# HudsonAlpha/rust-msbwt

Hardware: AMD Instinct MI355X
Metric: k-mer count queries/sec (whole node) (higher is better)
Workload: dtype u64

## Files before the change

### include/msbwt_hip.h

```cpp
#ifndef MSBWT_HIP_H
#define MSBWT_HIP_H

#include <stddef.h>
#include <stdint.h>

#ifdef __cplusplus
extern "C" {
#endif

#define MSBWT_VC_LEN 6
#define MSBWT_LETTER_BITS 3
#define MSBWT_NUMBER_BITS 5
#define MSBWT_NUM_POWER 32
#define MSBWT_MASK 0x07
#define MSBWT_COUNT_MASK 0x1F

#define MSBWT_OK 0
#define MSBWT_ERR_IO (-1)
#define MSBWT_ERR_UNEXPECTED_EOF (-2)
#define MSBWT_ERR_BAD_HEADER (-3)
#define MSBWT_ERR_INVALID_SYMBOL (-4)
#define MSBWT_ERR_INVALID_RANGE (-5)
#define MSBWT_ERR_HIP (-6)
#define MSBWT_ERR_NOT_LOADED (-7)
// ... 184 lines not shown
int msbwt_sparse_filter_bits(uint64_t tag, uint32_t *word, uint32_t *mask);
int msbwt_rle_set_query_length(msbwt_rle *bwt, int k);
int msbwt_rle_get_query_length(const msbwt_rle *bwt);
int msbwt_auto_sparse_max_depth(int query_length);
size_t msbwt_rle_download_sparse_table(const msbwt_rle *bwt, void *out_lines, size_t cap_bytes, void *out_side, size_t cap_side_bytes);
int msbwt_rle_set_presence_filter(msbwt_rle *bwt, int mode);
int msbwt_rle_get_presence_filter(const msbwt_rle *bwt);
int msbwt_rle_set_pair_index(msbwt_rle *bwt, int mode);
int msbwt_rle_get_pair_index(const msbwt_rle *bwt);
int msbwt_rle_set_pair_stride(msbwt_rle *bwt, int stride);
int msbwt_rle_get_pair_stride(const msbwt_rle *bwt);
double msbwt_rle_get_typical_range_width(const msbwt_rle *bwt);
int msbwt_auto_pair_stride(uint64_t total_symbols, uint64_t free_hbm_bytes, uint64_t hbm_total_bytes, double typical_width, int *stride);
int msbwt_rle_set_memory_budget(msbwt_rle *bwt, uint64_t bytes);
uint64_t msbwt_rle_get_memory_budget(const msbwt_rle *bwt);
int msbwt_auto_index_plan(uint64_t total_symbols, uint64_t free_hbm_bytes, uint64_t hbm_total_bytes, double typical_width, uint64_t budget_bytes,
                          int *pair_index, int *pair_stride, int *flat_depth, int *packed_depth, uint64_t *index_bytes);
int msbwt_run_build_fits_device(uint64_t total_symbols, uint64_t free_hbm_bytes);
int msbwt_rle_set_block_format(msbwt_rle *bwt, int format);
int msbwt_rle_get_block_format(const msbwt_rle *bwt);
int msbwt_rle_set_search_kernel(msbwt_rle *bwt, int mode);
int msbwt_rle_get_search_kernel(const msbwt_rle *bwt);
int msbwt_rle_search_kernel_for(const msbwt_rle *bwt, size_t k);
#define MSBWT_SEARCH_COUNTERS 16
int msbwt_rle_set_search_counters(msbwt_rle *bwt, int enabled);
int msbwt_rle_search_counters(const msbwt_rle *bwt, uint64_t *out, void *hip_stream);
int msbwt_rle_set_line_streaming(msbwt_rle *bwt, int mode);
int msbwt_rle_get_line_streaming(const msbwt_rle *bwt);
int msbwt_rle_probe_line_rate(const msbwt_rle *bwt, int which, double *lines_per_second);
uint64_t msbwt_rle_device_bytes(const msbwt_rle *bwt);
int msbwt_rle_kernel_time_ms(const msbwt_rle *bwt, double *avg_ms, uint64_t *launches);
int msbwt_rle_set_kernel_timing(msbwt_rle *bwt, int enabled);
int msbwt_rle_device_ordinal(const msbwt_rle *bwt);
const char *msbwt_rle_last_error(const msbwt_rle *bwt);
size_t msbwt_build_plane_blocks(const uint8_t *rle_bytes, size_t len, void *out_blocks, size_t cap_blocks,
                                uint64_t *out_total);
size_t msbwt_build_run_blocks(const uint8_t *rle_bytes, size_t len, void *out_blocks, size_t cap_blocks,
                              void *out_overflow, size_t cap_overflow, uint64_t *out_total, uint64_t *out_noverflow);
size_t msbwt_rle_download_blocks(const msbwt_rle *bwt, void *out_blocks, size_t cap_blocks);
const char *msbwt_version(void);

size_t msbwt_convert_to_vec(const uint8_t *ascii, size_t n, uint8_t *out, size_t cap);
int msbwt_save_bwt_numpy(const uint8_t *rle_bytes, size_t n, const char *utf8_path);
int msbwt_save_bwt_runs_numpy(const uint8_t *syms, const uint64_t *counts, size_t nruns,
                              const char *utf8_path);
void msbwt_convert_stoi(const uint8_t *ascii, size_t n, uint8_t *out_codes);
// ... 8 lines not shown
```

### include/msbwt_hip.hpp

```cpp
#pragma once

#include <algorithm>
#include <array>
#include <cstdint>
#include <stdexcept>
#include <string>
#include <system_error>
#include <vector>

#include "msbwt_hip.h"

namespace msbwt {

constexpr std::size_t VC_LEN = MSBWT_VC_LEN;
constexpr std::size_t LETTER_BITS = MSBWT_LETTER_BITS;
constexpr std::size_t NUMBER_BITS = MSBWT_NUMBER_BITS;
constexpr std::size_t NUM_POWER = MSBWT_NUM_POWER;
constexpr std::uint8_t MASK = MSBWT_MASK;
constexpr std::uint8_t COUNT_MASK = MSBWT_COUNT_MASK;

struct BWTRange {
    std::uint64_t l = 0;
    std::uint64_t h = 0;
    bool operator==(const BWTRange &o) const { return l == o.l && h == o.h; }
// ... 427 lines not shown
    }
    void device_status(void *hip_stream = nullptr) const { check(msbwt_rle_device_status(raw_, hip_stream)); }
    void allgather_counts(void *comm, const void *d_mine, std::size_t n_mine, void *d_all, int wire_bits = 64,
                          void *hip_stream = nullptr) const {
        check(msbwt_rle_allgather_counts(raw_, comm, d_mine, n_mine, d_all, wire_bits, hip_stream));
    }

    void set_table_depth(int depth) { check(msbwt_rle_set_table_depth(raw_, depth)); }
    void set_table_packed(int mode) { check(msbwt_rle_set_table_packed(raw_, mode)); }
    void set_pair_index(int mode) { check(msbwt_rle_set_pair_index(raw_, mode)); }
    void set_search_kernel(int mode) { check(msbwt_rle_set_search_kernel(raw_, mode)); }
    void set_memory_budget(std::uint64_t bytes) { check(msbwt_rle_set_memory_budget(raw_, bytes)); }
    void set_batch_order(int mode) { check(msbwt_rle_set_batch_order(raw_, mode)); }
    void set_sparse_table(int depth) { check(msbwt_rle_set_sparse_table(raw_, depth)); }
    void set_query_length(int k) { check(msbwt_rle_set_query_length(raw_, k)); }
    int get_query_length() const { return msbwt_rle_get_query_length(raw_); }
    void set_sparse_tiers(int mode) { check(msbwt_rle_set_sparse_tiers(raw_, mode)); }
    bool get_sparse_tiers() const { return msbwt_rle_get_sparse_tiers(raw_) != 0; }
    void set_sparse_second(int mode) { check(msbwt_rle_set_sparse_second(raw_, mode)); }
    int get_sparse_table() const { return msbwt_rle_get_sparse_table(raw_); }
    void set_table_side(int mode) { check(msbwt_rle_set_table_side(raw_, mode)); }
    std::uint64_t device_bytes() const { return msbwt_rle_device_bytes(raw_); }
    int search_kernel_for(size_t k) const { return msbwt_rle_search_kernel_for(raw_, k); }
    msbwt_rle *raw() const { return raw_; }

    RleBWT replicate(int device) const {
        msbwt_rle *other = msbwt_rle_replicate(raw_, device);
        if (!other) throw Panic(MSBWT_ERR_HIP, msbwt_rle_last_error(raw_));
        return RleBWT(other);
    }
    static std::vector<std::uint64_t> count_kmers_multi(const std::vector<const RleBWT *> &replicas,
                                                        const std::vector<std::uint8_t> &kmers, std::size_t k) {
        if (replicas.empty()) throw std::invalid_argument("no replicas");
        const std::size_t n = k ? kmers.size() / k : 0;
        std::vector<const msbwt_rle *> raws;
        for (const RleBWT *r : replicas) raws.push_back(r->raw_);
        std::vector<std::uint64_t> out(n);
        const int code = msbwt_rle_count_kmers_multi(raws.data(), raws.size(), kmers.data(), k, n, out.data());
        if (code != MSBWT_OK) throw Panic(code, "count_kmers_multi failed");
        return out;
    }

  private:
    explicit RleBWT(msbwt_rle *adopted) : raw_(adopted) {}
    void check(int code) const {
        if (code == MSBWT_OK) return;
// ... 61 lines not shown
```

### rust-msbwt_amd/_build.py

```python
import os
import subprocess
import sys

HERE = os.path.dirname(os.path.abspath(__file__))
CSRC = os.path.join(HERE, "csrc")
LIB = os.path.join(HERE, "libmsbwt_hip.so")
SOURCES = ["capi.cpp", "index_build.cpp", "query.cpp", "sources.cpp", "spectrum.cpp", "produce.cpp", "multi_device.cpp", "kernels.hip", "lanes.hip", "lanes_tier.hip", "lanes_wide.hip", "lanes_xwide.hip", "extend.hip", "sparse_table.hip", "device_build.hip", "pair_index.hip", "gather.hip", "order.hip", "run_build.hip", "reads_build.hip", "run_encode.hip", "merge.hip", "merge_many.hip", "source_index.hip", "spectrum.hip", "canonical.hip", "source_spectrum.hip", "kmer_graph.hip", "plane_index.cpp", "run_index.cpp", "npy_io.cpp", "rle_codec.cpp"]
HEADERS = ["handle.hpp", "index_build.hpp", "kernels.hpp", "lanes_kernel.hpp", "sparse_table.hpp", "sparse_build.hpp", "sparse_policy.hpp", "device_build.hpp", "pair_index.hpp", "gather.hpp", "order.hpp", "run_build.hpp", "reads_build.hpp", "run_encode.hpp", "workgroup.hpp", "rle_subruns.hpp", "merge.hpp", "merge_common.hpp", "source_index.hpp", "source_count.hpp", "source_spectrum.hpp", "kmer_graph.hpp", "frontier.hpp", "frontier_walk.hpp", "spectrum.hpp", "canonical.hpp", "rank_ops.hpp", "search_common.hpp", "host_pipeline.hpp", "plane_index.hpp", "run_index.hpp", "table_policy.hpp", "npy_io.hpp", "rle_codec.hpp", os.path.join("..", "..", "include", "msbwt_hip.h")]


def hipcc():
    for cand in (os.environ.get("HIPCC"), "/opt/rocm/bin/hipcc", "hipcc"):
        if cand and (os.path.isabs(cand) and os.path.exists(cand) or not os.path.isabs(cand)):
            return cand
    return "hipcc"


def stale():
    if not os.path.exists(LIB):
        return True
    t = os.path.getmtime(LIB)
    deps = [os.path.join(CSRC, f) for f in SOURCES + HEADERS] + [os.path.abspath(__file__)]
    return any(os.path.getmtime(d) > t for d in deps)


def build(force=False, verbose=False):
    if not force and not stale():
        return LIB
    from concurrent.futures import ThreadPoolExecutor

    objdir = os.path.join(HERE, "build")
# ... 31 lines not shown
```

### rust-msbwt_amd/_lib.py

```python
import ctypes as C
import os

HERE = os.path.dirname(os.path.abspath(__file__))
LIB_PATH = os.path.join(HERE, "libmsbwt_hip.so")

OK = 0
ERR_IO, ERR_UNEXPECTED_EOF, ERR_BAD_HEADER, ERR_INVALID_SYMBOL = -1, -2, -3, -4
ERR_INVALID_RANGE, ERR_HIP, ERR_NOT_LOADED, ERR_TOO_LARGE, ERR_INVALID_ARG, ERR_INTERNAL = -5, -6, -7, -8, -9, -10
ERR_OVERFLOW, ERR_RCCL = -11, -12
COMM_ID_BYTES = 128
SPARSE_INFO_WORDS = 120
BUILD_STAGES = ("copy_in", "read_order", "histogram", "collect", "sort", "emit", "encode", "copy_out")
MERGE_MAX_INPUTS = 32
SOURCE_INDEX_SLACK = 1024
SPECTRUM_INFO_WORDS = 40
SPECTRUM_MIN_FRONTIER = 64
MERGE_STAGES = ("copy_in", "decode", "iterate", "emit", "encode", "copy_out")

SIZE_MAX = C.c_size_t(-1).value

_vp, _u8, _u64, _sz, _int = C.c_void_p, C.c_uint8, C.c_uint64, C.c_size_t, C.c_int
_pu64 = C.POINTER(C.c_uint64)
SIGNATURES = {
    "msbwt_rle_new": (_vp, [_u8]),
# ... 87 lines not shown
    "msbwt_rle_get_memory_budget": (_u64, [_vp]),
    "msbwt_auto_index_plan": (_int, [_u64, _u64, _u64, C.c_double, _u64, C.POINTER(C.c_int), C.POINTER(C.c_int), C.POINTER(C.c_int), C.POINTER(C.c_int), _pu64]),
    "msbwt_rle_set_table_side": (_int, [_vp, _int]),
    "msbwt_rle_table_info": (_int, [_vp, _pu64, _pu64, _pu64]),
    "msbwt_rle_set_sparse_table": (_int, [_vp, _int]),
    "msbwt_rle_get_sparse_table": (_int, [_vp]),
    "msbwt_rle_sparse_table_info": (_int, [_vp, _pu64]),
    "msbwt_sparse_hash": (_int, [_u64, _int, _u64, C.POINTER(C.c_uint32), C.POINTER(C.c_uint32)]),
    "msbwt_sparse_table_shape": (_int, [_int, _u64, _pu64, C.POINTER(C.c_int)]),
    "msbwt_sparse_hash64": (_int, [_u64, _int, _u64, C.POINTER(C.c_uint32), _pu64]),
    "msbwt_auto_sparse_depth": (_int, [_pu64, _pu64, _int, _u64, _int, C.POINTER(C.c_int), _pu64]),
    "msbwt_rle_download_sparse_table": (_sz, [_vp, _vp, _sz, _vp, _sz]),
    "msbwt_allgather_piece_queries": (_sz, [_sz, _int]),
    "msbwt_rle_set_search_counters": (_int, [_vp, _int]),
    "msbwt_rle_search_counters": (_int, [_vp, _vp, _vp]),
    "msbwt_rle_set_presence_filter": (_int, [_vp, _int]),
    "msbwt_rle_get_presence_filter": (_int, [_vp]),
    "msbwt_run_build_fits_device": (_int, [_u64, _u64]),
    "msbwt_rle_set_block_format": (_int, [_vp, _int]),
    "msbwt_rle_get_block_format": (_int, [_vp]),
    "msbwt_rle_set_search_kernel": (_int, [_vp, _int]),
    "msbwt_rle_get_search_kernel": (_int, [_vp]),
    "msbwt_rle_search_kernel_for": (_int, [_vp, _sz]),
    "msbwt_rle_set_pair_index": (_int, [_vp, _int]),
    "msbwt_rle_get_pair_index": (_int, [_vp]),
    "msbwt_rle_set_pair_stride": (_int, [_vp, _int]),
    "msbwt_rle_get_pair_stride": (_int, [_vp]),
    "msbwt_rle_get_typical_range_width": (C.c_double, [_vp]),
    "msbwt_auto_pair_stride": (_int, [_u64, _u64, _u64, C.c_double, C.POINTER(C.c_int)]),
    "msbwt_rle_set_sparse_tiers": (_int, [_vp, _int]),
    "msbwt_rle_get_sparse_tiers": (_int, [_vp]),
    "msbwt_rle_set_sparse_second": (_int, [_vp, _int]),
    "msbwt_auto_sparse_choice": (_int, [_pu64, _pu64, _pu64, _int, _u64, _int, _int, C.POINTER(C.c_int), C.POINTER(C.c_int), _pu64]),
    "msbwt_sparse_filter_bits": (_int, [_u64, C.POINTER(C.c_uint32), C.POINTER(C.c_uint32)]),
    "msbwt_rle_set_query_length": (_int, [_vp, _int]),
    "msbwt_rle_get_query_length": (_int, [_vp]),
    "msbwt_auto_sparse_max_depth": (_int, [_int]),
    "msbwt_rle_set_line_streaming": (_int, [_vp, _int]),
    "msbwt_rle_get_line_streaming": (_int, [_vp]),
    "msbwt_rle_probe_line_rate": (_int, [_vp, _int, C.POINTER(C.c_double)]),
    "msbwt_rle_device_bytes": (_u64, [_vp]),
    "msbwt_rle_kernel_time_ms": (_int, [_vp, C.POINTER(C.c_double), _pu64]),
    "msbwt_rle_set_kernel_timing": (_int, [_vp, _int]),
    "msbwt_rle_device_ordinal": (_int, [_vp]),
    "msbwt_rle_last_error": (C.c_char_p, [_vp]),
    "msbwt_version": (C.c_char_p, []),
# ... 50 lines not shown
```

### rust-msbwt_amd/csrc/capi.cpp

```cpp
#include <algorithm>
#include <cstdint>
#include <cstdio>
#include <cstdlib>
#include <cstring>
#include <mutex>
#include <string>
#include <vector>

#include "handle.hpp"
#include "index_build.hpp"
#include "npy_io.hpp"
#include "pair_index.hpp"
#include "plane_index.hpp"
#include "run_index.hpp"
#include "sparse_table.hpp"

namespace {

constexpr int kMaxTableDepth = 16;
static_assert(MSBWT_SEARCH_COUNTERS == kSearchCounters, "the header's counter block is the kernels'");
static_assert(MSBWT_BUILD_STAGES == kReadsBuildStages, "the header's stage count is the builder's");
static_assert(MSBWT_MERGE_STAGES == kMergeStages, "the header's stage count is the merge's");
static_assert(MSBWT_MERGE_MAX_INPUTS == kMergeMaxInputs, "the header's input count is the merge's");
static_assert(10 + kSparseMaxDepth + 1 <= 42 && 45 + kSparseMaxDepth + 1 <= 80 && 80 + kSparseMaxDepth + 1 <= 112 && 119 <= MSBWT_SPARSE_INFO_WORDS,
              "msbwt_rle_sparse_table_info: [10 + d] distinct, [42] filtered, [45 + d] wide, [80 + d] once, [112] second tier, [113 .. 119) the walks");

const char *kVersion = "rust-msbwt_amd 0.1.0 (gfx950 plane-block index)";

double line_rate_of(const void *p, size_t bytes, hipStream_t stream) {
    hipEvent_t a = nullptr, b = nullptr;
    uint64_t lines = 0;
    float ms = 0.f;
    hipError_t e = hipEventCreate(&a);
    if (e == hipSuccess) e = hipEventCreate(&b);
    if (e == hipSuccess) e = launch_probe_lines(p, bytes, 4, nullptr, nullptr, stream);
    if (e == hipSuccess) e = hipEventRecord(a, stream);
    if (e == hipSuccess) e = launch_probe_lines(p, bytes, 48, &lines, nullptr, stream);
    if (e == hipSuccess) e = hipEventRecord(b, stream);
// ... 127 lines not shown
    if (device < 0 && hipGetDevice(&device) != hipSuccess) device = 0;
    h->device = device;
    if (const char *env = std::getenv("MSBWT_TABLE_DEPTH")) h->wanted_table_depth = std::max(-1, std::min(std::atoi(env), kMaxTableDepth));
    if (const char *env = std::getenv("MSBWT_TABLE_PACKED")) h->wanted_table_packed = std::atoi(env) ? 1 : 0;
    if (const char *env = std::getenv("MSBWT_TABLE_SIDE")) h->wanted_table_side = std::atoi(env) ? 1 : 0;
    if (const char *env = std::getenv("MSBWT_STREAM_LINES")) h->wanted_streaming = std::strcmp(env, "auto") == 0 ? -1 : (std::atoi(env) ? 1 : 0);
    if (const char *env = std::getenv("MSBWT_QUERY_K")) h->query_length = std::max(0, std::atoi(env));
    if (const char *env = std::getenv("MSBWT_SPARSE_TABLE")) {
        const int d = std::strcmp(env, "auto") == 0 ? -1 : std::atoi(env);
        h->wanted_sparse = (d == 0 || d == -1 || (d >= kSparseMinDepth && d <= kSparseMaxDepth)) ? d : -1;
    }
    if (const char *env = std::getenv("MSBWT_SPARSE_SECOND")) h->wanted_second = std::strcmp(env, "auto") == 0 ? -1 : (std::atoi(env) ? -1 : 0);
    if (const char *env = std::getenv("MSBWT_SPARSE_TIERS")) h->wanted_tiers = std::strcmp(env, "auto") == 0 ? -1 : (std::atoi(env) ? 1 : 0);
    if (const char *env = std::getenv("MSBWT_PAIR_INDEX")) h->wanted_pair = std::atoi(env) ? 1 : 0;
    if (const char *env = std::getenv("MSBWT_PAIR_STRIDE")) h->wanted_pair_stride = std::atoi(env);
    if (const char *env = std::getenv("MSBWT_FILTER")) h->wanted_filter = std::atoi(env) ? -1 : 0;
    if (const char *env = std::getenv("MSBWT_BLOCKS")) h->wanted_block_format = std::strcmp(env, "runs") == 0 ? kBlocksRuns : kBlocksPlanes;
    if (const char *env = std::getenv("MSBWT_MEMORY_BUDGET")) h->memory_budget = std::strtoull(env, nullptr, 10);
    if (const char *env = std::getenv("MSBWT_ORDER")) h->wanted_order = std::strcmp(env, "auto") == 0 ? -1 : (std::atoi(env) ? 1 : 0);
    if (const char *env = std::getenv("MSBWT_BUILD_PIECE")) h->build_piece = std::strtoull(env, nullptr, 10);
    if (const char *env = std::getenv("MSBWT_ORDER_BITS")) h->order_bits = std::max(1, std::min(std::atoi(env), 36));
    if (const char *env = std::getenv("MSBWT_SEARCH"))
        h->search_kernel = std::strcmp(env, "groups") == 0 ? kSearchGroups : std::strcmp(env, "lanes") == 0 ? kSearchLanes : kSearchAuto;
    return h;
}

msbwt_rle *msbwt_rle_new(uint8_t bin_power) { return msbwt_rle_new_on_device(bin_power, -1); }

void msbwt_rle_free(msbwt_rle *h) {
    if (!h) return;
    {
        DeviceScope scope(h->device);
        release_index(h);
        for (hipEvent_t e : h->events) (void)hipEventDestroy(e);
        for (auto &t : h->tickets) {
            if (t.done) (void)hipEventDestroy(t.done);
            if (t.counters) (void)hipFree(t.counters);
            if (t.order_scratch) (void)hipFree(t.order_scratch);
            if (t.range_scratch) (void)hipFree(t.range_scratch);
        }
        h->pipe.release();
        if (h->mail) (void)hipHostFree(h->mail);
        if (h->d_gather) (void)hipFree(h->d_gather);
        for (hipEvent_t e : h->piece_events) (void)hipEventDestroy(e);
        if (h->gather_stream) (void)hipStreamDestroy(h->gather_stream);
        if (h->d_stage) (void)hipFree(h->d_stage);
// ... 310 lines not shown
    const uint64_t bytes96 = wide.pair_block_bytes + wide.super_bytes + wide.scratch_bytes, bytes128 = narrow.pair_block_bytes + narrow.super_bytes;
    const uint64_t after128 = free_hbm_bytes > bytes128 ? free_hbm_bytes - bytes128 : 0;
    *stride = choose_pair_stride(bytes96, expected_table_bytes(total_symbols, nblocks * kBlockBytes, after128, true, true), free_hbm_bytes,
                                 hbm_total_bytes, typical_width);
    return MSBWT_OK;
}

double msbwt_rle_get_typical_range_width(const msbwt_rle *h) { return h ? h->typical_width : -1.0; }

int msbwt_rle_set_search_kernel(msbwt_rle *h, int mode) {
    if (!h || mode < kSearchAuto || mode > kSearchLanes) return MSBWT_ERR_INVALID_ARG;
    return set_locked(h, h->search_kernel, mode);
}

int msbwt_rle_get_search_kernel(const msbwt_rle *h) { return h ? h->search_kernel : 0; }

int msbwt_rle_search_kernel_for(const msbwt_rle *h, size_t k) {
    if (!h || !h->loaded) return MSBWT_ERR_INVALID_ARG;
    if (k > 0xFFFFFFFFull) return 0;
    Call c(h);
    return search_kernel_for(view_of(c.h), uint32_t(k));
}

uint64_t msbwt_rle_device_bytes(const msbwt_rle *h) {
    if (!h || !h->loaded) return 0;
    const DirectTable &t = h->table;
    return h->nblocks * kBlockBytes + h->overflow_bytes + (t.entries ? uint64_t(t.bytes) + t.side_bytes : 0) + h->pair.bytes +
           (t.filter ? (uint64_t(1) << (2 * t.filter_depth)) / 8 : 0) + h->sparse.bytes + h->sparse.side_bytes + h->sparse2.bytes + h->sparse2.side_bytes + h->sources.bytes;
}

int msbwt_rle_set_kernel_timing(msbwt_rle *h, int enabled) {
    return h ? set_locked(h, h->timing, enabled != 0) : MSBWT_ERR_INVALID_ARG;
}

int msbwt_rle_kernel_time_ms(const msbwt_rle *ch, double *avg_ms, uint64_t *launches) {
    Call c(ch);
    msbwt_rle *h = c.h;
    if (!h) return MSBWT_ERR_INVALID_ARG;
    if (int rc = c.bind()) return rc;
    const int rc = drain_timing_events(h);
    if (rc) return rc;
    if (avg_ms) *avg_ms = h->timed_launches ? h->timed_ms / double(h->timed_launches) : 0.0;
    if (launches) *launches = h->timed_launches;
    h->timed_ms = 0.0;
    h->timed_launches = 0;
    return MSBWT_OK;
// ... 77 lines not shown
```

### rust-msbwt_amd/csrc/handle.hpp

```cpp
#pragma once
#include <hip/hip_runtime_api.h>

#include <cstdio>
#include <cstdlib>
#include <mutex>
#include <optional>
#include <string>
#include <vector>

#include "../../include/msbwt_hip.h"
#include "host_pipeline.hpp"
#include "kernels.hpp"
#include "merge.hpp"
#include "plane_index.hpp"
#include "reads_build.hpp"
#include "rle_codec.hpp"
#include "sparse_build.hpp"
#include "source_index.hpp"
#include "sparse_policy.hpp"
#include "table_policy.hpp"

using namespace msbwt;

namespace msbwt_capi __attribute__((visibility("hidden"))) {
// ... 63 lines not shown
        if (rows) (void)hipFree(rows);
        if (checkpoints) (void)hipFree(checkpoints);
        *this = SourceIndex{};
    }
    SourceView view(uint64_t total) const {
        return SourceView{static_cast<const uint8_t *>(rows), static_cast<const uint64_t *>(checkpoints), total, n_sources, source_stride(n_sources)};
    }
};

struct Settings {
    int wanted_block_format = kBlocksPlanes;
    int wanted_pair = -1;
    int wanted_pair_stride = 0;
    int wanted_table_side = 1;
    int wanted_second = -1;
    int wanted_tiers = -1;
    int wanted_streaming = -1;
    int wanted_sparse = -1;
    int query_length = 0;
    int wanted_table_packed = -1;
    int wanted_filter = -1;
    int wanted_table_depth = -1;
    int search_kernel = kSearchAuto;
    int wanted_order = -1;
    int order_bits = 22;
    uint64_t build_piece = 0;
    uint64_t memory_budget = 0;
    bool planned = false;
    IndexPlan plan{};
};

}

using namespace msbwt_capi;

struct msbwt_rle : Settings {
    int device = 0;
    uint8_t bin_power = 8;
    bool loaded = false;
    Totals totals{};
    void *d_blocks = nullptr;
    uint64_t nblocks = 0;
    int block_format = kBlocksPlanes;
    void *d_overflow = nullptr;
    uint64_t overflow_bytes = 0;
    PairIndex pair;
// ... 235 lines not shown
```

### rust-msbwt_amd/csrc/query.cpp

```cpp
#include <algorithm>
#include <atomic>
#include <chrono>
#include <cstring>
#include <string>
#include <vector>

#include "gather.hpp"
#include "handle.hpp"
#include "order.hpp"

namespace {

constexpr size_t kMailQueries = 64, kMailKmerBytes = 4096;
constexpr size_t kMailDone = 0;
constexpr size_t kMailKmers = 64, kMailCounts = kMailKmers + kMailKmerBytes, kMailSyms = kMailCounts + 8 * kMailQueries,
                 kMailL = kMailSyms + 64, kMailH = kMailL + 8 * kMailQueries, kMailOutL = kMailH + 8 * kMailQueries,
                 kMailOutH = kMailOutL + 8 * kMailQueries, kMailBytes = kMailOutH + 8 * kMailQueries;

int ensure_mail(msbwt_rle *h) {
    if (int rc = ensure_runtime(h)) return rc;
    if (h->mail) return MSBWT_OK;
    void *host = nullptr, *dev = nullptr;
    HIP_TRY(h, hipHostMalloc(&host, kMailBytes, hipHostMallocMapped | hipHostMallocCoherent));
    const hipError_t e = hipHostGetDevicePointer(&dev, host, 0);
    if (e != hipSuccess) {
        (void)hipHostFree(host);
        return hip_fail(h, e, "hipHostGetDevicePointer");
    }
    std::memset(host, 0, kMailBytes);
    h->mail = static_cast<uint8_t *>(host);
    h->d_mail = static_cast<uint8_t *>(dev);
    return MSBWT_OK;
// ... 118 lines not shown
            const SourceView sv = h->sources.view(v.total);
            hipError_t e = hipSuccess;
            for (size_t first = 0; first < n && e == hipSuccess; first += kBySourcePiece) {
                const size_t m = std::min(kBySourcePiece, n - first);
                e = launch_kmer_ranges(v, d_kmers + first * k, uint32_t(k), m, pairs, pairs + 1, 2u, h->d_flags + which, stream);
                if (e == hipSuccess) e = launch_range_sources(sv, pairs, pairs + 1, 2u, m, d_out + first * sv.n_sources, h->d_flags + which, stream);
            }
            return e;
        });
    });
}

int launch_sources_of_ranges(msbwt_rle *h, const uint64_t *d_l, const uint64_t *d_h, size_t n, uint64_t *d_out, hipStream_t stream, int which) {
    return timed_launch(h, stream, [&] { return launch_range_sources(h->sources.view(h->totals.total), d_l, d_h, 1u, n, d_out, h->d_flags + which, stream); });
}

int need_sources(msbwt_rle *h) { return h->sources.n_sources ? int(MSBWT_OK) : fail(h, MSBWT_ERR_NOT_LOADED, "no sources attached"); }

size_t by_source_chunk(const msbwt_rle *h) { return std::min(size_t(1) << 21, (size_t(96) << 20) / (h->sources.n_sources * sizeof(uint64_t))); }

int launch_read_kmers_locked(msbwt_rle *h, const void *d_reads, size_t read_len, size_t n_reads, size_t k,
                                    int ascii, void *d_out_fwd, void *d_out_rc, hipStream_t stream, int which) {
    return timed_with_tickets(h, stream, [&](const IndexView &v) {
        return launch_count_read_kmers(v, static_cast<const uint8_t *>(d_reads), uint32_t(read_len), n_reads, uint32_t(k), ascii != 0,
                                       static_cast<uint64_t *>(d_out_fwd), static_cast<uint64_t *>(d_out_rc), h->d_flags + which, stream);
    });
}

HostArray host_in(const void *p, size_t item_bytes) { return HostArray{p, nullptr, item_bytes}; }
HostArray host_out(void *p, size_t item_bytes) { return HostArray{nullptr, p, item_bytes}; }

template <class Launch>
int run_host_batch(msbwt_rle *h, size_t n, size_t chunk, const std::vector<HostArray> &ins, const std::vector<HostArray> &outs, const char *what,
                   Launch &&launch) {
    int launch_rc = MSBWT_OK;
    const hipError_t e = h->pipe.run(n, chunk, ins, outs, h->stream, [&](size_t, size_t m, void *const *d_in, void *const *d_out, hipStream_t stream) {
        launch_rc = launch(m, d_in, d_out, stream);
        return launch_rc ? hipErrorUnknown : hipSuccess;
    });
    if (launch_rc) return launch_rc;
    if (e != hipSuccess) return hip_fail(h, e, (std::string(what) + " pipeline").c_str());
    return status_of(h, h->stream, kHostFlags);
}

template <class Launch, class CopyOut>
int mailbox_call(msbwt_rle *h, IndexView &v, bool poll, Launch &&launch, CopyOut &&copy_out) {
// ... 375 lines not shown
```

### rust-msbwt_amd/rle_bwt.py

```python
import ctypes as C
import os

import numpy as np

from . import _lib
from .msbwt_core import BWT, BWTRange, VC_LEN


class MsbwtError(Exception):
    def __init__(self, code, message=""):
        super().__init__("msbwt error %d: %s" % (code, message))
        self.code = code


def _raise(code, handle):
    msg = _lib.lib().msbwt_rle_last_error(handle)
    msg = msg.decode(errors="replace") if msg else ""
    if code in (_lib.ERR_IO, _lib.ERR_UNEXPECTED_EOF):
        err = EOFError(msg) if code == _lib.ERR_UNEXPECTED_EOF else OSError(msg)
        err.code = code
        raise err
    raise MsbwtError(code, msg)


# ... 767 lines not shown
        rc = _lib.lib().msbwt_rle_set_block_format(self._h, self.BLOCK_FORMATS.get(fmt, fmt))
        if rc:
            _raise(rc, self._h)

    def get_block_format(self):
        return {v: k for k, v in self.BLOCK_FORMATS.items()}[int(_lib.lib().msbwt_rle_get_block_format(self._h))]

    SEARCH_KERNELS = {"auto": 0, "groups": 1, "lanes": 2}

    def set_search_kernel(self, mode):
        rc = _lib.lib().msbwt_rle_set_search_kernel(self._h, self.SEARCH_KERNELS.get(mode, mode))
        if rc:
            _raise(rc, self._h)

    def get_search_kernel(self):
        return {v: k for k, v in self.SEARCH_KERNELS.items()}[int(_lib.lib().msbwt_rle_get_search_kernel(self._h))]

    def search_kernel_for(self, k):
        rc = int(_lib.lib().msbwt_rle_search_kernel_for(self._h, int(k)))
        if rc < 0:
            _raise(rc, self._h)
        return {0: "generic", 1: "groups", 2: "lanes"}[rc]

    def set_line_streaming(self, mode):
        rc = _lib.lib().msbwt_rle_set_line_streaming(self._h, int(mode))
        if rc:
            _raise(rc, self._h)

    def get_line_streaming(self):
        return bool(_lib.lib().msbwt_rle_get_line_streaming(self._h))

    PROBE_ARRAYS = {"blocks": 0, "pair_blocks": 1, "sparse_table": 2, "table": 3}

    def probe_line_rate(self, which):
        out = C.c_double()
        rc = _lib.lib().msbwt_rle_probe_line_rate(self._h, self.PROBE_ARRAYS.get(which, which), C.byref(out))
        if rc:
            _raise(rc, self._h)
        return float(out.value)

    def device_bytes(self):
        return int(_lib.lib().msbwt_rle_device_bytes(self._h))

    def set_kernel_timing(self, enabled):
        _lib.lib().msbwt_rle_set_kernel_timing(self._h, 1 if enabled else 0)

# ... 147 lines not shown
```

Measured before the change: 32.75 billion.

## Add fused read-window k-mer lookup kernel using sparse hash table

Adds a dedicated kernel for counting all k-mer windows of reads when k equals the sparse table depth. It stages and packs read bytes in LDS per wave, extracts each window's 2-bit key, and does a single hashed bucket lookup with async global-to-LDS line loads, software-pipelined against the next tile. The aim is to replace the per-window backward-search path with direct table hits. Windows containing invalid symbols fall back to the backward search. The cost is a large amount of new, complex code and a narrow set of conditions under which the kernel is used.

```diff
diff --git a/include/msbwt_hip.h b/include/msbwt_hip.h
--- a/include/msbwt_hip.h
+++ b/include/msbwt_hip.h
@@ -230,6 +230,8 @@
 int msbwt_rle_set_search_kernel(msbwt_rle *bwt, int mode);
 int msbwt_rle_get_search_kernel(const msbwt_rle *bwt);
 int msbwt_rle_search_kernel_for(const msbwt_rle *bwt, size_t k);
+int msbwt_rle_read_windows_kernel_for(const msbwt_rle *bwt, size_t k);
+int msbwt_read_windows_lookup_rule(int sparse_depth, int two_tier, size_t k, int ragged, int block_format, int counters, int search_kernel, int enabled);
 #define MSBWT_SEARCH_COUNTERS 16
 int msbwt_rle_set_search_counters(msbwt_rle *bwt, int enabled);
 int msbwt_rle_search_counters(const msbwt_rle *bwt, uint64_t *out, void *hip_stream);
diff --git a/include/msbwt_hip.hpp b/include/msbwt_hip.hpp
--- a/include/msbwt_hip.hpp
+++ b/include/msbwt_hip.hpp
@@ -473,6 +473,7 @@
     void set_table_side(int mode) { check(msbwt_rle_set_table_side(raw_, mode)); }
     std::uint64_t device_bytes() const { return msbwt_rle_device_bytes(raw_); }
     int search_kernel_for(size_t k) const { return msbwt_rle_search_kernel_for(raw_, k); }
+    int read_windows_kernel_for(size_t k) const { return msbwt_rle_read_windows_kernel_for(raw_, k); }
     msbwt_rle *raw() const { return raw_; }
 
     RleBWT replicate(int device) const {
diff --git a/rust-msbwt_amd/_build.py b/rust-msbwt_amd/_build.py
--- a/rust-msbwt_amd/_build.py
+++ b/rust-msbwt_amd/_build.py
@@ -5,8 +5,8 @@
 HERE = os.path.dirname(os.path.abspath(__file__))
 CSRC = os.path.join(HERE, "csrc")
 LIB = os.path.join(HERE, "libmsbwt_hip.so")
-SOURCES = ["capi.cpp", "index_build.cpp", "query.cpp", "sources.cpp", "spectrum.cpp", "produce.cpp", "multi_device.cpp", "kernels.hip", "lanes.hip", "lanes_tier.hip", "lanes_wide.hip", "lanes_xwide.hip", "extend.hip", "sparse_table.hip", "device_build.hip", "pair_index.hip", "gather.hip", "order.hip", "run_build.hip", "reads_build.hip", "run_encode.hip", "merge.hip", "merge_many.hip", "source_index.hip", "spectrum.hip", "canonical.hip", "source_spectrum.hip", "kmer_graph.hip", "plane_index.cpp", "run_index.cpp", "npy_io.cpp", "rle_codec.cpp"]
-HEADERS = ["handle.hpp", "index_build.hpp", "kernels.hpp", "lanes_kernel.hpp", "sparse_table.hpp", "sparse_build.hpp", "sparse_policy.hpp", "device_build.hpp", "pair_index.hpp", "gather.hpp", "order.hpp", "run_build.hpp", "reads_build.hpp", "run_encode.hpp", "workgroup.hpp", "rle_subruns.hpp", "merge.hpp", "merge_common.hpp", "source_index.hpp", "source_count.hpp", "source_spectrum.hpp", "kmer_graph.hpp", "frontier.hpp", "frontier_walk.hpp", "spectrum.hpp", "canonical.hpp", "rank_ops.hpp", "search_common.hpp", "host_pipeline.hpp", "plane_index.hpp", "run_index.hpp", "table_policy.hpp", "npy_io.hpp", "rle_codec.hpp", os.path.join("..", "..", "include", "msbwt_hip.h")]
+SOURCES = ["capi.cpp", "index_build.cpp", "query.cpp", "sources.cpp", "spectrum.cpp", "produce.cpp", "multi_device.cpp", "kernels.hip", "lanes.hip", "lanes_tier.hip", "lanes_wide.hip", "lanes_xwide.hip", "window_lookup.hip", "extend.hip", "sparse_table.hip", "device_build.hip", "pair_index.hip", "gather.hip", "order.hip", "run_build.hip", "reads_build.hip", "run_encode.hip", "merge.hip", "merge_many.hip", "source_index.hip", "spectrum.hip", "canonical.hip", "source_spectrum.hip", "kmer_graph.hip", "plane_index.cpp", "run_index.cpp", "npy_io.cpp", "rle_codec.cpp"]
+HEADERS = ["handle.hpp", "index_build.hpp", "kernels.hpp", "lanes_kernel.hpp", "window_lookup.hpp", "sparse_table.hpp", "sparse_build.hpp", "sparse_policy.hpp", "device_build.hpp", "pair_index.hpp", "gather.hpp", "order.hpp", "run_build.hpp", "reads_build.hpp", "run_encode.hpp", "workgroup.hpp", "rle_subruns.hpp", "merge.hpp", "merge_common.hpp", "source_index.hpp", "source_count.hpp", "source_spectrum.hpp", "kmer_graph.hpp", "frontier.hpp", "frontier_walk.hpp", "spectrum.hpp", "canonical.hpp", "rank_ops.hpp", "search_common.hpp", "host_pipeline.hpp", "plane_index.hpp", "run_index.hpp", "table_policy.hpp", "npy_io.hpp", "rle_codec.hpp", os.path.join("..", "..", "include", "msbwt_hip.h")]
 
 
 def hipcc():
diff --git a/rust-msbwt_amd/_lib.py b/rust-msbwt_amd/_lib.py
--- a/rust-msbwt_amd/_lib.py
+++ b/rust-msbwt_amd/_lib.py
@@ -133,6 +133,8 @@
     "msbwt_rle_set_search_kernel": (_int, [_vp, _int]),
     "msbwt_rle_get_search_kernel": (_int, [_vp]),
     "msbwt_rle_search_kernel_for": (_int, [_vp, _sz]),
+    "msbwt_rle_read_windows_kernel_for": (_int, [_vp, _sz]),
+    "msbwt_read_windows_lookup_rule": (_int, [_int, _int, _sz, _int, _int, _int, _int, _int]),
     "msbwt_rle_set_pair_index": (_int, [_vp, _int]),
     "msbwt_rle_get_pair_index": (_int, [_vp]),
     "msbwt_rle_set_pair_stride": (_int, [_vp, _int]),
diff --git a/rust-msbwt_amd/csrc/capi.cpp b/rust-msbwt_amd/csrc/capi.cpp
--- a/rust-msbwt_amd/csrc/capi.cpp
+++ b/rust-msbwt_amd/csrc/capi.cpp
@@ -14,6 +14,7 @@
 #include "plane_index.hpp"
 #include "run_index.hpp"
 #include "sparse_table.hpp"
+#include "window_lookup.hpp"
 
 namespace {
 
@@ -187,6 +188,7 @@
     if (const char *env = std::getenv("MSBWT_ORDER_BITS")) h->order_bits = std::max(1, std::min(std::atoi(env), 36));
     if (const char *env = std::getenv("MSBWT_SEARCH"))
         h->search_kernel = std::strcmp(env, "groups") == 0 ? kSearchGroups : std::strcmp(env, "lanes") == 0 ? kSearchLanes : kSearchAuto;
+    if (const char *env = std::getenv("MSBWT_WINDOW_LOOKUP")) h->window_lookup = std::atoi(env) ? 1 : 0;
     return h;
 }
 
@@ -543,6 +545,18 @@
     return search_kernel_for(view_of(c.h), uint32_t(k));
 }
 
+int msbwt_rle_read_windows_kernel_for(const msbwt_rle *h, size_t k) {
+    if (!h || !h->loaded) return MSBWT_ERR_INVALID_ARG;
+    if (k > 0xFFFFFFFFull) return 0;
+    Call c(h);
+    const IndexView v = view_of(c.h);
+    return window_lookup_serves(v, k, false, c.h->window_lookup != 0) ? kSearchLookup : search_kernel_for(v, uint32_t(k));
+}
+
+int msbwt_read_windows_lookup_rule(int sparse_depth, int two_tier, size_t k, int ragged, int block_format, int counters, int search_kernel, int enabled) {
+    return window_lookup_rule(sparse_depth, two_tier != 0, k, ragged != 0, block_format, counters != 0, search_kernel, enabled != 0) ? 1 : 0;
+}
+
 uint64_t msbwt_rle_device_bytes(const msbwt_rle *h) {
     if (!h || !h->loaded) return 0;
     const DirectTable &t = h->table;
diff --git a/rust-msbwt_amd/csrc/handle.hpp b/rust-msbwt_amd/csrc/handle.hpp
--- a/rust-msbwt_amd/csrc/handle.hpp
+++ b/rust-msbwt_amd/csrc/handle.hpp
@@ -109,6 +109,7 @@
     int wanted_filter = -1;
     int wanted_table_depth = -1;
     int search_kernel = kSearchAuto;
+    int window_lookup = 1;
     int wanted_order = -1;
     int order_bits = 22;
     uint64_t build_piece = 0;
diff --git a/rust-msbwt_amd/csrc/query.cpp b/rust-msbwt_amd/csrc/query.cpp
--- a/rust-msbwt_amd/csrc/query.cpp
+++ b/rust-msbwt_amd/csrc/query.cpp
@@ -8,6 +8,7 @@
 #include "gather.hpp"
 #include "handle.hpp"
 #include "order.hpp"
+#include "window_lookup.hpp"
 
 namespace {
 
@@ -172,6 +173,9 @@
 int launch_read_kmers_locked(msbwt_rle *h, const void *d_reads, size_t read_len, size_t n_reads, size_t k,
                                     int ascii, void *d_out_fwd, void *d_out_rc, hipStream_t stream, int which) {
     return timed_with_tickets(h, stream, [&](const IndexView &v) {
+        if (window_lookup_serves(v, k, false, h->window_lookup != 0))
+            return launch_count_read_windows(v, static_cast<const uint8_t *>(d_reads), uint32_t(read_len), n_reads, uint32_t(k), ascii != 0,
+                                             static_cast<uint64_t *>(d_out_fwd), static_cast<uint64_t *>(d_out_rc), h->d_flags + which, stream);
         return launch_count_read_kmers(v, static_cast<const uint8_t *>(d_reads), uint32_t(read_len), n_reads, uint32_t(k), ascii != 0,
                                        static_cast<uint64_t *>(d_out_fwd), static_cast<uint64_t *>(d_out_rc), h->d_flags + which, stream);
     });
diff --git a/rust-msbwt_amd/csrc/window_lookup.hip b/rust-msbwt_amd/csrc/window_lookup.hip
--- /dev/null
+++ b/rust-msbwt_amd/csrc/window_lookup.hip
@@ -0,0 +1,323 @@
+#include "window_lookup.hpp"
+
+#include "lanes_kernel.hpp"
+
+namespace msbwt {
+namespace {
+
+constexpr uint32_t kWinStageAt = region_base(8);
+constexpr uint32_t kWinLines = kWinStageAt + 64u;
+constexpr uint32_t kWinTwoWords = 132, kWinMaskWords = 68;
+static_assert((kWinTwoWords + kWinMaskWords) * 4u <= 1024u, "the staging area is the ninth region");
+static_assert(kWinLines * 16u <= 160u * 1024u / 16u, "16 one-wave workgroups per CU");
+constexpr uint32_t kWinMaxK = 31;
+constexpr int kWinWavesPerCu = 16;
+
+struct WindowLaunch {
+    const uint4 *table, *side, *blocks;
+    const uint8_t *reads;
+    uint64_t *out_fwd, *out_rc;
+    uint32_t *flags;
+    uint64_t total, n_windows, step_reads;
+    uint32_t step_windows, nbuckets, probe, read_len, windows, k, strands, ascii, stream_lines;
+};
+
+template <uint32_t kTagBits>
+__host__ __device__ constexpr SparseLayout window_layout() {
+    return kTagBits == 40u ? kLayoutXwide : kTagBits == 32u ? kLayoutWide : kLayoutComplete;
+}
+
+__device__ __forceinline__ uint32_t ascii_dword(uint32_t x) {
+    return ascii_to_code(x & 0xFFu) | (ascii_to_code((x >> 8) & 0xFFu) << 8) | (ascii_to_code((x >> 16) & 0xFFu) << 16) | (ascii_to_code(x >> 24) << 24);
+}
+
+__device__ __forceinline__ void pack_codes(uint32_t x, uint32_t &codes, uint32_t &flagged) {
+    const uint32_t invalid = ((x + 0x7A7A7A7Au) | x) & 0x80808080u;
+    const uint32_t low2 = x & 0x03030303u;
+    const uint32_t none = (low2 - 0x01010101u) & ~low2 & 0x80808080u;
+    const uint32_t bad = ((invalid | none) >> 7) & 0x01010101u, spread = bad * 0xFFu;
+    const uint32_t y = ((x & 0x07070707u) & ~spread) | (0x01010101u & spread);
+    const uint32_t c = y - 0x01010101u - ((y >> 2) & 0x01010101u);
+    codes = (c * 0x40100401u) >> 24;
+    flagged = (bad * 0x08040201u) >> 24;
+}
+
+__device__ __forceinline__ void pack_piece(uint4 v, bool ascii, uint32_t &word, uint32_t &mask16) {
+    if (ascii) v = make_uint4(ascii_dword(v.x), ascii_dword(v.y), ascii_dword(v.z), ascii_dword(v.w));
+    uint32_t c0, c1, c2, c3, f0, f1, f2, f3;
+    pack_codes(v.x, c0, f0);
+    pack_codes(v.y, c1, f1);
+    pack_codes(v.z, c2, f2);
+    pack_codes(v.w, c3, f3);
+    word = (c0 << 24) | (c1 << 16) | (c2 << 8) | c3;
+    mask16 = (f0 << 12) | (f1 << 8) | (f2 << 4) | f3;
+}
+
+__device__ __forceinline__ uint64_t revcomp_key(uint64_t key, uint32_t k) {
+    uint64_t r = __brevll(key) >> (64u - 2u * k);
+    r = ((r >> 1) & 0x5555555555555555ull) | ((r & 0x5555555555555555ull) << 1);
+    return r ^ ((1ull << (2u * k)) - 1ull);
+}
+
+__device__ __forceinline__ int nth_set_lane(uint64_t mask, uint32_t group, uint64_t *rest) {
+    int src = -1;
+#pragma unroll
+    for (uint32_t j = 0; j < 8u; ++j) {
+        const int b = mask != 0ull ? __ffsll(static_cast<unsigned long long>(mask)) - 1 : -1;
+        if (j == group) src = b;
+        mask &= mask - 1ull;
+    }
+    *rest = mask;
+    return src;
+}
+
+struct WindowUnit {
+    uint64_t win;
+    uint64_t first;
+    uint64_t fkey;
+    uint64_t want;
+    uint32_t bucket;
+    bool valid, flagged, rc;
+};
+
+template <uint32_t kTagBits>
+__global__ __launch_bounds__(64) __attribute__((amdgpu_waves_per_eu(4, 4))) void k_count_kmers_windows(const WindowLaunch a) {
+    constexpr SparseLayout L = window_layout<kTagBits>();
+    __shared__ uint4 lines[kWinLines];
+    const uint32_t lane = threadIdx.x, group = lane >> 3, sub = lane & 7u, k = a.k, n = 2u * k;
+    const uint32_t chunk_bytes = (sub ^ group) * 16u;
+    const uint64_t ntiles = (a.n_windows + 63u) / 64u, nwaves = gridDim.x;
+    uint32_t *two = reinterpret_cast<uint32_t *>(&lines[kWinStageAt]);
+    uint32_t *mk = two + kWinTwoWords;
+    uint16_t *mk16 = reinterpret_cast<uint16_t *>(mk);
+
+    uint64_t tile = blockIdx.x, read0 = (blockIdx.x * 64u) / a.windows;
+    uint32_t win0 = (blockIdx.x * 64u) % a.windows;
+
+    auto stage = [&](WindowUnit &u) {
+        const uint64_t g0 = tile * 64u;
+        const uint32_t in_tile = uint32_t(min(uint64_t(64), a.n_windows - g0));
+        const uint32_t at = win0 + min(lane, in_tile - 1u);
+        const uint32_t q = a.windows >= 64u ? (at >= a.windows ? 1u : 0u) : at / a.windows;
+        const uint32_t rel = q * a.read_len + (at - q * a.windows) - win0;
+        const uint64_t b0 = read0 * a.read_len + win0;
+        const uintptr_t start = reinterpret_cast<uintptr_t>(a.reads) + b0;
+        const uint32_t lead = uint32_t(start) & 15u;
+        const uint32_t nbytes = lead + uint32_t(__builtin_amdgcn_readlane(int(rel), 63)) + k;
+        const uint32_t pieces = (nbytes + 15u) >> 4;
+        const uint4 *src = reinterpret_cast<const uint4 *>(start - lead);
+        wave_lds_sync();
+#pragma unroll
+        for (uint32_t half = 0; half < 2u; ++half) {
+            const uint32_t p = lane + 64u * half;
+            if (half * 64u < pieces) {
+                if (p < pieces) {
+                    uint32_t word, mask16;
+                    pack_piece(src[p], a.ascii != 0u, word, mask16);
+                    two[p] = word;
+                    mk16[p ^ 1u] = uint16_t(mask16);
+                }
+            }
+        }
+        wave_lds_sync();
+        const uint32_t s = lead + rel, wi = s >> 4, o = 2u * (s & 15u);
+        const uint64_t top = (uint64_t(two[wi]) << 32) | two[wi + 1u];
+        const uint64_t cut = (top << o) | ((uint64_t(two[wi + 2u]) << o) >> 32);
+        const uint64_t flags64 = (uint64_t(mk[s >> 5]) << 32) | mk[(s >> 5) + 1u];
+        u.fkey = cut >> (64u - n);
+        u.flagged = ((flags64 << (s & 31u)) >> (64u - k)) != 0ull;
+        u.valid = lane < in_tile;
+        u.win = g0 + min(lane, in_tile - 1u);
+        u.first = b0 + rel;
+        wave_lds_sync();
+    };
+    auto aim = [&](WindowUnit &u, bool rc) {
+        u.rc = rc;
+        const uint64_t x = sparse_mix(rc ? revcomp_key(u.fkey, k) : u.fkey, n);
+        u.bucket = sparse_bucket(x, n, a.nbuckets);
+        u.want = (uint64_t(sparse_tag_hi(x, L)) << 32) | sparse_tag(x, L);
+    };
+    auto fetch_region = [&](uint32_t region, uint32_t bucket_of_src) {
+        const uintptr_t addr = reinterpret_cast<uintptr_t>(a.table) + uint64_t(bucket_of_src) * 128u + chunk_bytes;
+        if (a.stream_lines) __builtin_amdgcn_global_load_lds((global_void *)addr, (lds_void *)&lines[region_base(region)], 16, 0, 2);
+        else __builtin_amdgcn_global_load_lds((global_void *)addr, (lds_void *)&lines[region_base(region)], 16, 0, 0);
+    };
+    auto fetch_tile = [&](const WindowUnit &u) {
+        const bool looking = u.valid && !u.flagged;
+        const uint64_t look = __ballot(looking);
+        const uint32_t mine = looking ? u.bucket : 0u;
+        uint32_t b[8];
+#pragma unroll
+        for (uint32_t i = 0; i < 8u; ++i) b[i] = uint32_t(__shfl(int(mine), int(8u * i + group)));
+        __builtin_amdgcn_s_waitcnt(0xC07F);
+        wave_lds_sync();
+#pragma unroll
+        for (uint32_t i = 0; i < 8u; ++i)
+            if (((look >> (8u * i)) & 0xFFull) != 0ull) fetch_region(i, b[i]);
+    };
+    auto lines_landed = [&] {
+        __builtin_amdgcn_s_waitcnt(0);
+        wave_lds_sync();
+    };
+    auto store = [&](const WindowUnit &u, uint64_t value) { (u.rc ? a.out_rc : a.out_fwd)[u.win] = value; };
+
+    const bool both = a.strands == 3u;
+    auto advance = [&](bool was_rc) -> bool {
+        if (both && !was_rc) return false;
+        tile += nwaves;
+        read0 += a.step_reads;
+        win0 += a.step_windows;
+        if (win0 >= a.windows) {
+            win0 -= a.windows;
+            ++read0;
+        }
+        return true;
+    };
+
+    if (tile >= ntiles) return;
+    WindowUnit cur;
+    stage(cur);
+    aim(cur, a.strands == 2u);
+    fetch_tile(cur);
+    for (bool more = true; more;) {
+        WindowUnit next = cur;
+        const bool staged = advance(cur.rc);
+        more = tile < ntiles;
+        if (more) {
+            if (staged) stage(next);
+            aim(next, both ? !staged : a.strands == 2u);
+        }
+        lines_landed();
+        const bool looking = cur.valid && !cur.flagged;
+        uint64_t l = 0, count = 0;
+        uint32_t width = 0, header = 0, dist = 0, bucket = cur.bucket;
+        bool maybe = false, onward = false, escape = false;
+        if (looking) {
+            if (sparse_scan<L.slots>(lines, lane, L, cur.want, l, width, header, maybe)) {
+                count = width;
+                escape = width == kSparseEscapeWidth;
+            } else {
+                onward = header > L.slots && dist < a.probe;
+            }
+        }
+        if (more) fetch_tile(next);
+        for (uint64_t todo = __ballot(onward); todo != 0ull;) {
+            const uint32_t rank = __builtin_amdgcn_mbcnt_hi(uint32_t(todo >> 32), __builtin_amdgcn_mbcnt_lo(uint32_t(todo), 0u));
+            const bool riding = onward && rank < 8u;
+            if (riding) {
+                ++bucket;
+                ++dist;
+            }
+            uint64_t rest;
+            const int src = nth_set_lane(todo, group, &rest);
+            const uint32_t b = uint32_t(__shfl(int(bucket), src < 0 ? 0 : src));
+            __builtin_amdgcn_s_waitcnt(0xC07F);
+            wave_lds_sync();
+            fetch_region(8u, src < 0 ? 0u : b);
+            lines_landed();
+            if (riding) {
+                if (sparse_scan<L.slots>(lines, 64u + rank, L, cur.want, l, width, header, maybe)) {
+                    count = width;
+                    escape = width == kSparseEscapeWidth;
+                    onward = false;
+                } else {
+                    onward = header > L.slots && dist < a.probe;
+                }
+            }
+            todo = __ballot(onward);
+        }
+        if (__ballot(escape) != 0ull) {
+            if (escape) {
+                const uint4 e = a.side[l];
+                count = ((uint64_t(e.w) << 32) | e.z) - ((uint64_t(e.y) << 32) | e.x);
+            }
+        }
+        if (looking) store(cur, count);
+        for (uint64_t todo = __ballot(cur.valid && cur.flagged); todo != 0ull;) {
+            uint64_t rest;
+            const int src = nth_set_lane(todo, group, &rest);
+            todo = rest;
+            const int from = src < 0 ? 0 : src;
+            const uint64_t first = (uint64_t(uint32_t(__shfl(int(uint32_t(cur.first >> 32)), from))) << 32) | uint32_t(__shfl(int(uint32_t(cur.first)), from));
+            const uint64_t win = (uint64_t(uint32_t(__shfl(int(uint32_t(cur.win >> 32)), from))) << 32) | uint32_t(__shfl(int(uint32_t(cur.win)), from));
+            if (src < 0) continue;
+            const uint8_t *bytes = a.reads + first;
+            auto code_at = [&](uint32_t i) -> uint32_t { return a.ascii ? ascii_to_code(bytes[i]) : uint32_t(bytes[i]); };
+            uint32_t bad = 0;
+            for (uint32_t i = sub; i < k; i += kGroup) bad |= code_at(i) >= 6u ? 1u : 0u;
+            bad = group_sum(bad);
+            uint64_t result;
+            if (bad) {
+                result = ~0ull;
+                if (sub == 0u) atomicOr(a.flags, kFlagInvalidSymbol);
+            } else {
+                Range r{0, a.total};
+                bool broken = false;
+                for (uint32_t t = 0; t < k && r.l != r.h && !(broken = r.h > a.total || r.l > r.h); ++t) {
+                    const uint32_t s = cur.rc ? complement_code(code_at(t)) : code_at(k - 1u - t);
+                    r = constrain(a.blocks, s, r.l, r.h, sub);
+                }
+                result = broken ? ~0ull : r.h - r.l;
+                if (broken && sub == 0u) atomicOr(a.flags, kFlagInternal);
+            }
+            if (sub == 0u) (cur.rc ? a.out_rc : a.out_fwd)[win] = result;
+        }
+        cur = next;
+    }
+}
+
+template <uint32_t kTagBits>
+uint32_t resident_window_waves() {
+    static const uint32_t cached = [] {
+        int device = 0, cus = 0, per_cu = 0;
+        if (hipGetDevice(&device) != hipSuccess || hipDeviceGetAttribute(&cus, hipDeviceAttributeMultiprocessorCount, device) != hipSuccess ||
+            hipOccupancyMaxActiveBlocksPerMultiprocessor(&per_cu, k_count_kmers_windows<kTagBits>, 64, 0) != hipSuccess || cus <= 0 || per_cu <= 0)
+            return uint32_t(kWinWavesPerCu) * 256u;
+        per_cu = std::min(per_cu, kWinWavesPerCu);
+        if (per_cu > 4) per_cu -= per_cu % 4;
+        if (std::getenv("MSBWT_VERBOSE")) std::fprintf(stderr, "[msbwt] window lookup kernel <%u>: %d workgroups per CU x %d CUs\n", kTagBits, per_cu, cus);
+        return uint32_t(cus) * uint32_t(per_cu);
+    }();
+    return cached;
+}
+
+template <uint32_t kTagBits>
+hipError_t launch_windows(WindowLaunch a, hipStream_t stream) {
+    const uint64_t tiles = (a.n_windows + 63u) / 64u;
+    const uint64_t waves = std::min<uint64_t>(tiles, resident_window_waves<kTagBits>());
+    a.step_reads = (waves * 64u) / a.windows;
+    a.step_windows = uint32_t((waves * 64u) % a.windows);
+    hipLaunchKernelGGL(k_count_kmers_windows<kTagBits>, dim3(uint32_t(waves)), dim3(64), 0, stream, a);
+    return hipGetLastError();
+}
+
+}
+
+hipError_t launch_count_read_windows(const IndexView &ix, const uint8_t *reads, uint32_t read_len, uint64_t n_reads, uint32_t k, bool ascii,
+                                     uint64_t *out_fwd, uint64_t *out_rc, uint32_t *flags, hipStream_t stream) {
+    if (!window_lookup_serves(ix, k, false, true) || k > kWinMaxK || k > read_len || (!out_fwd && !out_rc)) return hipErrorInvalidValue;
+    if (n_reads == 0) return hipSuccess;
+    const SparseView &sp = *sparse_for(ix, k);
+    WindowLaunch a{};
+    a.table = static_cast<const uint4 *>(sp.lines);
+    a.side = static_cast<const uint4 *>(sp.side);
+    a.blocks = static_cast<const uint4 *>(ix.blocks);
+    a.reads = reads;
+    a.out_fwd = out_fwd;
+    a.out_rc = out_rc;
+    a.flags = flags;
+    a.total = ix.total;
+    a.nbuckets = sp.nbuckets;
+    a.probe = sp.probe;
+    a.read_len = read_len;
+    a.windows = read_len - k + 1u;
+    a.n_windows = n_reads * a.windows;
+    a.k = k;
+    a.strands = (out_fwd ? 1u : 0u) | (out_rc ? 2u : 0u);
+    a.ascii = ascii ? 1u : 0u;
+    a.stream_lines = ix.stream_lines ? 1u : 0u;
+    const uint32_t bits = sparse_tag_bits(sp.depth);
+    return bits == 40u ? launch_windows<40u>(a, stream) : bits == 32u ? launch_windows<32u>(a, stream) : launch_windows<24u>(a, stream);
+}
+
+}
diff --git a/rust-msbwt_amd/csrc/window_lookup.hpp b/rust-msbwt_amd/csrc/window_lookup.hpp
--- /dev/null
+++ b/rust-msbwt_amd/csrc/window_lookup.hpp
@@ -0,0 +1,23 @@
+#pragma once
+#include <cstdint>
+
+#include "kernels.hpp"
+
+namespace msbwt {
+
+constexpr int kSearchLookup = 3;
+
+inline bool window_lookup_rule(int sparse_depth, bool two_tier, uint64_t k, bool ragged, int block_format, bool counters, int search_kernel, bool enabled) {
+    return enabled && !ragged && !counters && !two_tier && search_kernel == kSearchAuto && block_format == kBlocksPlanes && sparse_depth >= kSparseMinDepth &&
+           sparse_depth <= kSparseMaxDepth && k == uint64_t(sparse_depth);
+}
+
+inline bool window_lookup_serves(const IndexView &ix, uint64_t k, bool ragged, bool enabled) {
+    const SparseView *sp = k <= 0xFFFFFFFFull ? sparse_for(ix, uint32_t(k)) : nullptr;
+    return sp != nullptr && window_lookup_rule(int(sp->depth), sp->tier != 0u, k, ragged, ix.block_format, ix.counters != nullptr, ix.search_kernel, enabled);
+}
+
+hipError_t launch_count_read_windows(const IndexView &ix, const uint8_t *reads, uint32_t read_len, uint64_t n_reads, uint32_t k, bool ascii,
+                                     uint64_t *out_fwd, uint64_t *out_rc, uint32_t *flags, hipStream_t stream);
+
+}
diff --git a/rust-msbwt_amd/rle_bwt.py b/rust-msbwt_amd/rle_bwt.py
--- a/rust-msbwt_amd/rle_bwt.py
+++ b/rust-msbwt_amd/rle_bwt.py
@@ -813,6 +813,12 @@
             _raise(rc, self._h)
         return {0: "generic", 1: "groups", 2: "lanes"}[rc]
 
+    def read_windows_kernel_for(self, k):
+        rc = int(_lib.lib().msbwt_rle_read_windows_kernel_for(self._h, int(k)))
+        if rc < 0:
+            _raise(rc, self._h)
+        return {0: "generic", 1: "groups", 2: "lanes", 3: "lookup"}[rc]
+
     def set_line_streaming(self, mode):
         rc = _lib.lib().msbwt_rle_set_line_streaming(self._h, int(mode))
         if rc:
```

Result: slower. 32.15 billion (-1.8%).
